# vainglorygame/analyzer

Hardware: AMD Instinct MI355X
Metric: matches/sec rated (whole node), 3v3 TrueSkill, 1M-player roster (higher is better)
Workload: dtype fp32; 1 GPU; global_batch=10000000, seq_len=6, players=1000000, matches_per_gpu=10000000, team_size=3, parallelism=dp1, mode=exact, bench_config=2, skew=1, force_merge=False

## Files before the change

### analyzer_amd/config.py

```python
from __future__ import annotations

import os
from dataclasses import dataclass, field
from typing import Mapping, Optional

BETA = 10.0 / 30 * 3000
ENV_MU = 1500.0
ENV_SIGMA = 1000.0
DRAW_PROBABILITY = 0.0

MODES = ("casual", "ranked", "blitz", "br", "5v5_casual", "5v5_ranked")
TRACK_COLUMNS = ("trueskill",) + tuple("trueskill_" + m for m in MODES)
N_TRACKS = len(TRACK_COLUMNS)
MODE_UNSUPPORTED = 255


def _env(env: Mapping[str, str], key: str) -> Optional[str]:
    v = env.get(key)
    return v if v else None


def _tristate(v: Optional[str]) -> Optional[bool]:
    if v is None or v == "" or v.lower() == "auto":
        return None
# ... 38 lines not shown
    crunch_queue: str = "crunch_global"
    dotelesuckmatch: bool = False
    telesuck_queue: str = "telesuck"
    dosewmatch: bool = False
    sew_queue: str = "sew"
    engine: str = "python"
    quarantine: bool = True
    dotelemetry: bool = False
    telemetry_events: str = "100,300"
    resident: bool = True
    synthetic_telemetry: bool = False
    telemetry_source: Optional[str] = None
    skip_rated: bool = False
    pipeline: bool = False
    fault_poison: frozenset = frozenset()
    fault_exit_after: int = 0
    cas_retries: int = 50

    @staticmethod
    def from_env(env: Mapping[str, str] = os.environ) -> "WorkerConfig":
        return WorkerConfig(
            rabbitmq_uri=_env(env, "RABBITMQ_URI") or "amqp://localhost",
            database_uri=_env(env, "DATABASE_URI"),
            batchsize=int(_env(env, "BATCHSIZE") or 500),
            chunksize=int(_env(env, "CHUNKSIZE") or 100),
            idle_timeout=float(_env(env, "IDLE_TIMEOUT") or 1),
            queue=_env(env, "QUEUE") or "analyze",
            docrunchmatch=env.get("DOCRUNCHMATCH") == "true",
            crunch_queue=_env(env, "CRUNCH_QUEUE") or "crunch_global",
            dotelesuckmatch=env.get("DOTELESUCKMATCH") == "true",
            telesuck_queue=_env(env, "TELESUCK_QUEUE") or "telesuck",
            dosewmatch=env.get("DOSEWMATCH") == "true",
            sew_queue=_env(env, "SEW_QUEUE") or "sew",
            engine=_env(env, "ENGINE") or "python",
            quarantine=(env.get("QUARANTINE") or "true") == "true",
            dotelemetry=env.get("DOTELEMETRY") == "true",
            telemetry_events=_env(env, "TELEMETRY_EVENTS") or "100,300",
            synthetic_telemetry=env.get("SYNTHETIC_TELEMETRY") == "true",
            telemetry_source=_env(env, "TELEMETRY_SOURCE"),
            resident=_resident_default(env),
            skip_rated=env.get("SKIP_RATED") == "true",
            pipeline=env.get("PIPELINE") == "true",
            fault_poison=frozenset(x for x in (env.get("FAULT_POISON") or "").split(",") if x),
            fault_exit_after=int(env.get("FAULT_EXIT_AFTER") or 0),
            cas_retries=int(env.get("CAS_RETRIES") or 50),
        )

    @property
    def failed_queue(self) -> str:
        return self.queue + "_failed"


@dataclass(frozen=True)
class EngineConfig:

    rate_blocks: int = 0
    prepass_at: float = 0.7
    prepass_at_set: bool = False
    prepass_cus: int = 0
    prepass_exclusive: bool = False
    prepass_serial: Optional[bool] = None
    roster_warm: Optional[bool] = None
    merge_bucket_mb: float = 64.0
    comm_dtype: str = ""
    sweeps: int = 1
    dist_backend: str = "nccl"
    checkpoint_every: int = 1
    checkpoint_dir: Optional[str] = None
    trace: bool = False
    check_rounds: bool = False
    rate_idle: int = 0
    rate_local: int = 1
    rate_diag: int = 0
    rate_tight: int = -1
    tele_fused_tail: int = 0
    tele_role: int = -1
    tele_fuse_max: int = 262_144

    NATIVE_KNOBS = {
        "ANA_TELE_IMPL": "telemetry aggregation: 1 one-hot MFMA GEMM (default), 0 LDS atomics",
        "ANA_SCHED_SMALL": "micro-batch schedule: hash lists (default) or bitonic sort",
        "ANA_SORT_RB / ANA_SORT_NT": "radix-sort tile rows / non-temporal loads (tuning)",
        "ANA_SCHED_RUNS": "last schedule pass: run-end table (1, default) or digit offsets + fix-up (0)",
    }

    def rate_knobs(self) -> list:
        return [self.rate_idle, self.rate_local, self.rate_diag, self.rate_tight, self.tele_fused_tail,
                self.tele_role]

    @staticmethod
    def from_env(env: Mapping[str, str] = os.environ) -> "EngineConfig":
        return EngineConfig(
            rate_blocks=int(_env(env, "ANA_RATE_BLOCKS") or 0),
            prepass_at=float(_env(env, "ANA_PREPASS_AT") or 0.7) if env.get("ANA_PREPASS_AT") != "0" else 0.0,
            prepass_at_set=bool(env.get("ANA_PREPASS_AT")),
            prepass_cus=int(_env(env, "ANA_PREPASS_CUS") or 0),
            prepass_exclusive=env.get("ANA_PREPASS_EXCLUSIVE", "0") not in ("", "0", "false"),
            prepass_serial=_tristate(env.get("ANA_PREPASS_SERIAL")),
            roster_warm=_tristate(env.get("ANA_ROSTER_WARM")),
            merge_bucket_mb=float(_env(env, "ANA_MERGE_BUCKET_MB") or 64),
            comm_dtype=_env(env, "COMM_DTYPE") or "",
            sweeps=int(_env(env, "SWEEPS") or 1),
            dist_backend=_env(env, "ANA_DIST_BACKEND") or "nccl",
            checkpoint_every=int(_env(env, "CHECKPOINT_EVERY") or 1),
            checkpoint_dir=_env(env, "CHECKPOINT_DIR"),
            trace=(env.get("ANA_TRACE") or "0") not in ("", "0"),
            check_rounds=(env.get("ANA_CHECK_ROUNDS") or "0") not in ("", "0"),
            rate_idle=int(_env(env, "ANA_RATE_IDLE") or 0),
            rate_local=int(_env(env, "ANA_RATE_LOCAL") or 1),
            rate_diag=int(_env(env, "ANA_RATE_DIAG") or 0),
            rate_tight=int(_env(env, "ANA_RATE_TIGHT") or -1),
            tele_fused_tail=int(_env(env, "ANA_TELE_FUSED_TAIL") or 0),
            tele_role=int(_env(env, "ANA_TELE_ROLE") or -1),
            tele_fuse_max=int(_env(env, "ANA_TELE_FUSE_MAX") or 262_144),
        )
```

### analyzer_amd/csrc/bindings.cpp

```cpp
#include <torch/extension.h>

#include <cstdlib>
#include <ATen/hip/HIPContext.h>

#include <algorithm>
#include <numeric>
#include <string>
#include <tuple>
#include <vector>

#include "career_core.h"
#include "common.h"
#include "gen_core.h"
#include "host.h"
#include "ingest.h"
#include "kernels.h"
#include "ladder_core.h"
#include "matchmake_core.h"
#include "select_core.h"

namespace {

using torch::Tensor;

// ... 948 lines not shown
  Tensor records = torch::empty({L, 2 * K + 2}, lobbies.options());
  if (L == 0) return {out, records};
  if (dev.is_cuda()) {
    check_hip(ana::launch_balance((int)K, lobbies.data_ptr<int32_t>(), L, state.data_ptr<float>(), at,
                                  vst.data_ptr<float>(), P, (int)mode, (float)beta2, (float)unknown_sigma,
                                  out.data_ptr<int32_t>(), records.data_ptr<int32_t>(), stream_of(lobbies)),
              "balance");
  } else {
    TORCH_CHECK(ana::host_balance((int)K, lobbies.data_ptr<int32_t>(), L, state.data_ptr<float>(), at,
                                  vst.data_ptr<float>(), P, (int)mode, (float)beta2, (float)unknown_sigma,
                                  out.data_ptr<int32_t>(), records.data_ptr<int32_t>()) == 0,
                "balance: bad arguments");
  }
  return {out, records};
}

std::vector<Tensor> queue_order(Tensor queue, Tensor state, c10::optional<Tensor> attrs, Tensor vst, int64_t mode,
                                double unknown_sigma) {
  const auto dev = queue.device();
  check(queue, "queue", torch::kInt32, dev);
  TORCH_CHECK(queue.dim() == 1 && queue.size(0) <= 0x7fffffffLL, "queue_order: queue must be [Q], Q < 2^31");
  TORCH_CHECK(mode >= 0 && mode < ana::kModes, "queue_order: mode must be 0..5");
  const float* at = matchmake_roster(state, attrs, vst, dev, "queue_order");
  const int64_t Q = queue.size(0), P = state.size(0);
  Tensor keys = torch::empty({Q}, queue.options()), vals = torch::empty({Q}, queue.options());
  if (Q == 0) return {keys, vals};
  if (!dev.is_cuda()) {
    TORCH_CHECK(ana::host_queue_keys(queue.data_ptr<int32_t>(), Q, state.data_ptr<float>(), at,
                                     vst.data_ptr<float>(), P, (int)mode, (float)unknown_sigma, u32p(keys),
                                     u32p(vals)) == 0, "queue_order: bad arguments");
    Tensor sk = torch::empty({Q}, queue.options()), sv = torch::empty({Q}, queue.options());
    const uint32_t* k = u32p(keys);
    uint32_t* order = u32p(sv);
    std::iota(order, order + Q, 0u);
    std::stable_sort(order, order + Q, [&](uint32_t a, uint32_t b) { return k[a] < k[b]; });
    for (int64_t i = 0; i < Q; ++i) u32p(sk)[i] = k[order[i]];
    return {sk, sv};
  }
  const hipStream_t s = stream_of(queue);
  check_hip(ana::launch_queue_keys(queue.data_ptr<int32_t>(), Q, state.data_ptr<float>(), at, vst.data_ptr<float>(),
                                   P, (int)mode, (float)unknown_sigma, u32p(keys), u32p(vals), s),
            "queue_keys");
  return sort_pairs_on_stream(keys, vals, Q, 32, s);
}

std::tuple<int64_t, int64_t, int64_t> matchmake_geometry(int64_t K) {
  TORCH_CHECK(K >= 1 && K <= ana::kMaxTeamSize, "matchmake_geometry: K must be 1..5");
  const int G = ana::split_group_lanes((int)K);
  return {G, 64 / G, ana::kMatchmakeThreads / G};
}

std::vector<int64_t> split_masks(int64_t K) {
  TORCH_CHECK(K >= 1 && K <= ana::kMaxTeamSize, "split_masks: K must be 1..5");
  std::vector<int64_t> out;
  ana::with_team_size((int)K, [&](auto k) {
    for (uint16_t m : ana::kSplits<decltype(k)::value>.mask) out.push_back(m);
  });
  return out;
}

void reset_tags(Tensor state) {
  const auto dev = state.device();
  const int64_t P = check_state(state, dev, "reset_tags");
  if (dev.is_cuda()) check_hip(ana::launch_reset_tags(state.data_ptr<float>(), P, stream_of(state)), "reset_tags");
  else ana::host_reset_tags(state.data_ptr<float>(), P);
}

}

void register_batch_host(pybind11::module& m);
void register_telemetry_file(pybind11::module& m);

PYBIND11_MODULE(TORCH_EXTENSION_NAME, m) {
  register_batch_host(m);
  register_telemetry_file(m);
  m.doc() = "analyzer_amd native engine: gfx950 HIP kernels + C++ host mirror";
  m.def("gen_roster", &gen_roster, "K7: synthetic roster (state [P,16], attrs [P,4])");
  m.def("gen_stream", &gen_stream, "K7: synthetic match stream rec [M, 2K+2]");
  m.def("schedule_workspace_bytes", &schedule_workspace_bytes);
  m.def("levels_device", &levels_device);
  m.def("sort_pairs", &sort_pairs, "stable LSD radix sort of int32 (key, value) pairs (device)");
  m.def("levels", &levels, "K5 host levelizer: per-match conflict-free round (0 = stateless)");
  m.def("schedule", &schedule, "K5: per-slot occurrence index (chronological order per player)");
  m.def("rate", &rate, "K1-K4/K6: exact dataflow rating of a stream");
  m.def("gen_event_counts", &gen_event_counts, "K8/K7: synthetic telemetry events per match");
  m.def("gen_events", &gen_events, "K8/K7: synthetic telemetry events (CSR by match)");
  m.def("telemetry", &telemetry, "K8: per-participant telemetry aggregation [M, 2K, 8]");
  m.attr("STAT_FEATURES") = ana::kStatFeatures;
  m.def("sweep_delta", &sweep_delta, "K9: per-rank natural-parameter messages for the DP merge");
  m.def("sweep_apply", &sweep_apply, "K9: decode summed messages against the common start (-> s, s2)",
        py::arg("s0"), py::arg("buf"), py::arg("attrs"), py::arg("s"), py::arg("s2"), py::arg("vst"),
        py::arg("unknown_sigma"), py::arg("scaled"), py::arg("clamps") = py::none());
  m.def("sweep_delta_packed", &sweep_delta_packed, "K9: messages straight into bf16/fp16 + int32 all-reduce operands");
  m.def("sweep_apply_packed", &sweep_apply_packed,
        "K9: decode bf16/fp16 + int32 summed messages (-> s, s2); with a prefix also the record-correction delta table",
        py::arg("s0"), py::arg("msg"), py::arg("cnt"), py::arg("attrs"), py::arg("s"), py::arg("s2"), py::arg("vst"),
        py::arg("unknown_sigma"), py::arg("clamps") = py::none(), py::arg("prefix") = py::none(),
        py::arg("delta") = py::none());
  m.def("correct_records", &correct_records,
        "K9: causal correction of a window's records: += the delta table of the earlier ranks' messages");
  m.def("sweep_block_reduce", &sweep_block_reduce, "K9: owner block sum (+ exclusive prefixes) of the split collective",
        py::arg("recv"), py::arg("N"), py::arg("bf16"), py::arg("total"), py::arg("pref") = py::none());
  m.def("prefix_delta", &prefix_delta, "K9: the record correction's delta table of a scaled message prefix");
  m.def("pack_rows", &pack_rows, "C2: changed rows of a round slice -> fixed-capacity [cap, 33] entries");
  m.def("check_round", &check_round, "C2 race detector: one round's matches share no player (flag |= 1)");
  m.def("unpack_rows", &unpack_rows, "C2: write gathered entries (id >= 0) into the roster, tags zeroed");
  m.def("write_record_file", &write_record_file, "P3: write a match-record file (ANAREC01)");
  py::class_<ana::RecordReader>(m, "RecordReader")
      .def(py::init<const std::string&, int64_t, int, bool>(), py::arg("path"), py::arg("window"),
           py::arg("slots") = 3, py::arg("pinned") = true)
      .def_property_readonly("K", &ana::RecordReader::K)
      .def_property_readonly("num_matches", &ana::RecordReader::num_matches)
      .def_property_readonly("window", &ana::RecordReader::window)
      .def_property_readonly("num_windows", &ana::RecordReader::num_windows)
      .def_property_readonly("pinned", &ana::RecordReader::pinned)
      .def("acquire", &reader_acquire,
           "next filled window as (slot, base, tensor view of pinned memory) or None at EOF")
      .def("release", &ana::RecordReader::release, "return the oldest acquired slot");
  m.def("cu_masked_stream", &cu_masked_stream, "HIP stream limited to N CUs (spread over XCDs), or to the others",
        py::arg("device"), py::arg("num_cus"), py::arg("invert") = false);
  m.def("progress_signal", &progress_signal, "8-B signal-memory word for the executor's tail signal");
  m.def("stream_wait_value64", &stream_wait_value64, "hipStreamWaitValue64(stream, ptr, >= value)");
  m.def("stream_write_value64", &stream_write_value64, "hipStreamWriteValue64(stream, ptr, value)");
  m.def("can_wait_value", &can_wait_value, "hipDeviceAttributeCanUseStreamWaitValue");
  m.def("reset_tags", &reset_tags, "zero the dataflow tags of a roster");
  m.def("records_digest", &records_digest, "deterministic fp64 digest of a window's packed output rows "
        "(+ its status counts added to hist)", py::arg("rows"), py::arg("K"), py::arg("scratch"),
        py::arg("out"), py::arg("hist") = py::none());
  m.def("records_digest_scratch", &records_digest_scratch, "scratch doubles of records_digest");
  m.def("records_select", &records_select, "K10: hits [n, 12] int32 of the bitmap's players in a window's records "
        "joined with its packed output rows, ascending (match, slot)", py::arg("rec"), py::arg("rows"),
        py::arg("base"), py::arg("P"), py::arg("bitmap"));
  m.def("ladder", &ladder, "K11: [order, score, rank] per track of the mask (bit t = granule t) of a roster's state: "
        "descending score, ties by ascending id, rank -1 = unranked", py::arg("state"), py::arg("mask"),
        py::arg("score"), py::arg("max_sigma"));
  m.def("preview", &preview, "K12: packed [M, 4] int32 rows (status, quality, p_win0 bits, 0) of a stream's records "
        "against the stored roster: what rate would write, read-only", py::arg("rec"), py::arg("K"), py::arg("state"),
        py::arg("attrs"), py::arg("vst"), py::arg("beta2"), py::arg("unknown_sigma"));
  m.def("balance", &balance, "K12: [packed [L, 8] int32 rows (status, split, team0, quality, p_win0, quality_given), "
        "records [L, 2K+2]] of the best split of each lobby", py::arg("lobbies"), py::arg("K"), py::arg("state"),
        py::arg("attrs"), py::arg("vst"), py::arg("mode"), py::arg("beta2"), py::arg("unknown_sigma"));
  m.def("queue_order", &queue_order, "K12: [sorted keys, queue positions] of a queue by descending mode-track prior mu "
        "(stable; failed players last with key -1)", py::arg("queue"), py::arg("state"), py::arg("attrs"),
        py::arg("vst"), py::arg("mode"), py::arg("unknown_sigma"));
  m.def("matchmake_geometry", &matchmake_geometry, "K12: (lanes per lobby, lobbies per wave, lobbies per workgroup)");
  m.def("split_masks", &split_masks, "K12: the team-0 masks of the splits of a 2K lobby, in index order");
  m.def("careers_add", &careers_add, "K13: fold one window (rec [M, 2K+2] joined with its packed rows [M, W]) into the "
        "career table [P, 16] int32 in place: careers_add(table, rec, rows, base, P, track, score, modes)");
  m.attr("CAREER_WORDS") = ana::kCareerWords;
  m.attr("CAREER_TILE") = ana::kCareerTile;
  m.attr("MAX_SLOTS") = (int64_t)ana::kMaxSlots;
  m.attr("LADDER_CONSERVATIVE") = (int)ana::kLadderConservative;
  m.attr("LADDER_MU") = (int)ana::kLadderMu;
  m.attr("HIT_WORDS") = ana::kHitWords;
  m.attr("SELECT_TILE") = ana::kSelectTile;
  m.def("emulate_allreduce", &emulate_allreduce,
        "DP pricing on one GPU: an all-reduce stand-in (buffer unchanged) on N CUs for >= us microseconds");
  m.def("warm_rows", &warm_rows, "read every roster row once (cache warm-up before a rating launch)");
  m.def("epoch_bump", &epoch_bump, "device launch epoch += 1 (graph replays)");
  m.attr("ROW_FLOATS") = ana::kRowFloats;
  m.attr("N_TRACKS") = ana::kTracks;
  m.attr("VST_TIERS") = ana::kVstTiers;
}
```

### analyzer_amd/csrc/kernels.h

```cpp
#pragma once

#include <stddef.h>
#include <stdint.h>

#include <hip/hip_runtime_api.h>

#include "common.h"
#include "gen_core.h"
#include "telemetry_core.h"

namespace ana {

int launch_gen_roster(const GenRosterParams& g, float* state, float* attrs, hipStream_t s);
int launch_gen_stream(int K, const GenStreamParams& g, int32_t* rec, int64_t M, hipStream_t s);

int launch_reset_tags(float* state, int64_t P, hipStream_t s);
int launch_warm_rows(const float* state, int64_t P, uint32_t* sink, hipStream_t s);
int launch_epoch_bump(int32_t* e, hipStream_t s);
int launch_emulate_allreduce(void* buf, int64_t bytes, int channels, int passes, double us, hipStream_t s);

size_t schedule_workspace_bytes(int64_t nslots, int64_t num_players);

size_t records_digest_scratch_doubles(int K);
int launch_records_digest(int K, const float* rows, int64_t M, int64_t W, double* scratch, double* out,
                          int64_t* hist, hipStream_t s);

constexpr int kSelectTile = 2048;
int64_t records_select_tiles(int64_t M);
int launch_records_select_count(int K, const int32_t* rec, const float* rows, int64_t W, int64_t M, int64_t P,
                                const uint32_t* bitmap, uint32_t* counts, int64_t* offsets, hipStream_t s);
int launch_records_select_emit(int K, const int32_t* rec, const float* rows, int64_t W, int64_t M, int64_t base,
                               int64_t P, const uint32_t* bitmap, const int64_t* offsets, int32_t* hits,
                               int64_t nhits, hipStream_t s);

constexpr int kLadderTile = 1024;
int launch_ladder_keys(const float* state, int64_t P, uint32_t mask, int score, float max_sigma, uint32_t* keys,
                       uint32_t* ids, int64_t stride, uint32_t* counts, hipStream_t s);
int launch_ladder_ranks(const uint32_t* keys, const uint32_t* ids, int64_t P, int64_t R, int32_t* order, float* score,
                        int32_t* rank, hipStream_t s);

int launch_preview(int K, const int32_t* rec, int64_t M, const float* state, const float* attrs, const float* vst,
                   int64_t P, float beta2, float unknown_sigma, int32_t* out, hipStream_t s);
int launch_balance(int K, const int32_t* lobbies, int64_t L, const float* state, const float* attrs,
                   const float* vst, int64_t P, int mode, float beta2, float unknown_sigma, int32_t* out,
                   int32_t* records, hipStream_t s);
int launch_queue_keys(const int32_t* queue, int64_t Q, const float* state, const float* attrs, const float* vst,
                      int64_t P, int mode, float unknown_sigma, uint32_t* keys, uint32_t* vals, hipStream_t s);

constexpr int kCareerTile = 4096;
size_t career_edge_bytes(int64_t n);
int launch_career_keys(int K, const int32_t* rec, const float* rows, int64_t W, int64_t M, int64_t P, int track,
                       int score, uint32_t modes, uint32_t* keys, uint32_t* vals, uint32_t* events, hipStream_t s);
int launch_career_fold(const uint32_t* keys, const uint32_t* vals, const uint32_t* events, int64_t n, int K,
                       int64_t base, int64_t P, int32_t* table, void* edges, hipStream_t s);

size_t radix_sort_workspace_bytes(int64_t n);
int launch_radix_sort_pairs(uint32_t* keys, uint32_t* vals, uint32_t* keys_alt, uint32_t* vals_alt,
                            int64_t n, int bits, void* ws, int* result_in_alt, hipStream_t s);
int launch_sched_sort(int K, const int32_t* rec, int64_t M, uint32_t num_players, uint32_t* ka,
                      uint32_t* va, uint32_t* kb, uint32_t* vb, void* ws, uint32_t* link,
                      hipStream_t s, int32_t* deps = nullptr, uint32_t* ctrl = nullptr, int nz = 0,
                      int32_t* epoch_bump = nullptr, int sort_nt = -1);
int launch_levels(int K, const int32_t* rec, const uint32_t* link, int32_t* deps, int32_t* pushed,
                  int32_t* level, int64_t M, int64_t P, uint32_t* ctrl, hipStream_t s);
int launch_schedule(int K, const int32_t* rec, int64_t M, int64_t P, uint32_t* link,
                    int32_t* deps, void* ws, size_t ws_bytes, uint32_t* overflow, hipStream_t s,
                    bool zero_ctrl = false, int32_t* epoch_bump = nullptr, int sort_nt = -1);

int launch_rate(int K, const int32_t* rec, const uint32_t* link, int32_t* deps, float* state,
                const float* attrs, float* first_prior, const RateOut& out, uint32_t* ctrl,
                const RateParams& prm, const TelemetryParams& tp, int blocks, hipStream_t s);


int launch_gen_event_counts(const GenEventParams& g, int64_t base, int64_t M, int64_t* counts,
                            hipStream_t s);
int launch_gen_events(int K, const GenEventParams& g, int64_t base, const int32_t* rec,
                      const int64_t* evoff, int64_t M, int32_t* events, hipStream_t s);
int tele_impl();
int launch_telemetry(int K, const TelemetryParams& tp, uint32_t* bad, hipStream_t s);

}

namespace ana {
int launch_sweep_delta(const float* s0, const float* a, const float* s, const float* attrs,
                       const float* vst, float unknown_sigma, int scaled, float* buf, int64_t P,
                       hipStream_t st);
int launch_sweep_apply(const float* s0, const float* buf, const float* attrs, float* s, float* s2,
                       const float* vst, float unknown_sigma, int scaled, int64_t P, uint32_t* clamps,
                       hipStream_t st);
int launch_sweep_delta_packed(const float* s0, const float* a, const float* s, const float* attrs,
                              const float* vst, float unknown_sigma, int bf16, void* msg, int32_t* cnt,
                              int64_t P, hipStream_t st, int64_t mstride = 7, int64_t cstride = 1);
int launch_sweep_block_reduce(const int32_t* recv, int N, int64_t blk, int bf16, int32_t* total, int32_t* pref,
                              hipStream_t st);
int launch_sweep_apply_packed(const float* s0, const void* msg, const int32_t* cnt, int bf16,
                              const float* attrs, float* s, float* s2, const float* vst, float unknown_sigma,
                              int64_t P, uint32_t* clamps, const void* prefix, float* delta, hipStream_t st,
                              int64_t mstride = 7, int64_t cstride = 1);
int launch_prefix_delta(const float* s0, const void* prefix, int bf16, const float* attrs, const float* vst,
                        float unknown_sigma, float* delta, int64_t P, hipStream_t st);
int launch_correct_records(int K, const int32_t* rec, int64_t M, float* rows, int64_t orow, const float* delta,
                           int64_t P, hipStream_t st);
int launch_pack_rows(const int32_t* rec, int K, int64_t m, const uint8_t* status, int64_t sstride,
                     const float* state, float* out, int64_t cap, hipStream_t st);
int launch_unpack_rows(const float* buf, int64_t n, float* state, hipStream_t st);
int launch_check_round(const int32_t* rec, int K, const int64_t* idx, int64_t m, int64_t P, uint32_t round,
                       unsigned long long* owner, uint32_t* flag, hipStream_t st);
}
```

### analyzer_amd/csrc/radix_sort.hip

```cpp
#include <hip/hip_runtime.h>

#include <cstdlib>

#include "common.h"
#include "kernels.h"

namespace ana {

namespace {

#ifndef ANA_SORT_THREADS
#define ANA_SORT_THREADS 512
#endif
constexpr int kThreads = ANA_SORT_THREADS;
constexpr int kWaves = kThreads / 64;
constexpr int kItems = 16;
constexpr int kTile = kThreads * kItems;
constexpr int kRadix = 256;
constexpr int kRadixMax = 1024;

__device__ __forceinline__ int64_t xcd_tile(int64_t tiles) {
  const int64_t i = blockIdx.x, q = tiles >> 3, r = tiles & 7, x = i & 7;
  return x * q + (x < r ? x : r) + (i >> 3);
}

template <int NT>
__device__ __forceinline__ uint32_t ld32(const uint32_t* p) {
  if constexpr (NT >= 1) return __builtin_nontemporal_load(p);
  else return *p;
}
template <int NT>
__device__ __forceinline__ void st32(uint32_t* p, uint32_t v) {
  if constexpr (NT == 1) __builtin_nontemporal_store(v, p);
  else *p = v;
}

__device__ __forceinline__ uint32_t block_exclusive_scan(uint32_t x, uint32_t* wsum,
                                                         uint32_t* total) {
  const int lane = threadIdx.x & 63, wv = threadIdx.x >> 6;
  uint32_t inc = x;
#pragma unroll
  for (int off = 1; off < 64; off <<= 1) {
    const uint32_t y = __shfl_up(inc, off);
    if (lane >= off) inc += y;
  }
  if (lane == 63) wsum[wv] = inc;
  __syncthreads();
  uint32_t before = 0, all = 0;
#pragma unroll
  for (int w = 0; w < kWaves; ++w) {
    if (w < wv) before += wsum[w];
    all += wsum[w];
  }
  if (total) *total = all;
  __syncthreads();
  return before + inc - x;
}

template <int KS>
__device__ __forceinline__ void decode_tile_keys(const int32_t* __restrict__ rec, uint32_t kend,
                                                 int64_t base, int64_t n, uint32_t* lk) {
  constexpr int S = 2 * KS, R = S + 2;
  const uint32_t lo = (uint32_t)base;
  const uint32_t hi = (uint32_t)(base + kTile < n ? base + kTile : n);
  const uint32_t m_lo = lo / S, m_hi = (hi + S - 1) / S;
  for (uint32_t m = m_lo + threadIdx.x; m < m_hi; m += kThreads) {
    const int32_t* src = rec + (int64_t)m * R;
    int32_t r[R];
    if constexpr (R % 4 == 0) {
#pragma unroll
      for (int k = 0; k < R / 4; ++k) {
        const int4 v = reinterpret_cast<const int4*>(src)[k];
        r[4 * k] = v.x; r[4 * k + 1] = v.y; r[4 * k + 2] = v.z; r[4 * k + 3] = v.w;
      }
    } else {
#pragma unroll
      for (int k = 0; k < R; ++k) r[k] = src[k];
    }
    const bool rates = early_status<KS>(r, (int64_t)kend) == kRated;
    const uint32_t m0 = (uint32_t)r[S];
#pragma unroll
    for (int j = 0; j < S; ++j) {
      const uint32_t slot = m * S + j;
      const int pos = j < KS ? j : j - KS;
      const bool in_roster = pos < (j < KS ? meta_n0(m0) : meta_n1(m0));
      if (slot >= lo && slot < hi) lk[slot - lo] = rates && in_roster ? (uint32_t)r[j] : kend;
    }
  }
}

struct SchedInit {
  int32_t* deps = nullptr;
  uint32_t* ctrl = nullptr;
  int nz = 0;
  int32_t* epoch_bump = nullptr;
};

template <int KS, int RB = 8, int NT = 0>
__global__ void __launch_bounds__(kThreads)
radix_upsweep(const uint32_t* __restrict__ keys, const int32_t* __restrict__ rec, uint32_t kend,
              int64_t n, int shift, uint32_t* __restrict__ counts, int64_t tiles, SchedInit init = {}) {
  constexpr int kR = 1 << RB;
  __shared__ uint32_t hist[kWaves][kR];
  __shared__ uint32_t lkeys[KS > 0 ? kTile : 1];
  const int tid = threadIdx.x, wv = tid >> 6;
  for (int i = tid; i < kWaves * kR; i += kThreads) (&hist[0][0])[i] = 0u;
  const int64_t tile = xcd_tile(tiles);
  const int64_t base = tile * kTile;
  if constexpr (KS > 0) {
    if (init.deps) {
      constexpr int S = 2 * KS;
      const int64_t hi = base + kTile < n ? base + kTile : n;
      for (int64_t m = (base + S - 1) / S + tid; m < (hi + S - 1) / S; m += kThreads) init.deps[m] = 0;
    }
    if (blockIdx.x == 0) {
      if (tid < init.nz) init.ctrl[tid] = 0u;
      if (tid == 0 && init.epoch_bump) init.epoch_bump[0] += 1;
    }
  }
  if constexpr (KS > 0) decode_tile_keys<KS>(rec, kend, base, n, lkeys);
  __syncthreads();
#pragma unroll
  for (int k = 0; k < kItems; ++k) {
    const int64_t idx = base + k * kThreads + tid;
    if (idx < n) {
      const uint32_t key = KS > 0 ? lkeys[k * kThreads + tid] : ld32<NT>(keys + idx);
      atomicAdd(&hist[wv][(key >> shift) & (kR - 1)], 1u);
    }
  }
  __syncthreads();
#pragma unroll
  for (int d = tid; d < kR; d += kThreads) {
    uint32_t c = 0;
#pragma unroll
    for (int w = 0; w < kWaves; ++w) c += hist[w][d];
    counts[(int64_t)d * tiles + tile] = c;
  }
}

template <int DPT>
__device__ __forceinline__ void digits_exclusive_scan(uint32_t (&v)[DPT], uint32_t* wsum,
                                                      uint32_t* total) {
  uint32_t s = 0;
#pragma unroll
  for (int j = 0; j < DPT; ++j) {
    const uint32_t x = v[j];
    v[j] = s;
    s += x;
  }
  const uint32_t before = block_exclusive_scan(s, wsum, total);
#pragma unroll
  for (int j = 0; j < DPT; ++j) v[j] += before;
}

__global__ void __launch_bounds__(kThreads)
radix_rowscan(uint32_t* __restrict__ counts, int64_t tiles, uint32_t* __restrict__ totals) {
  __shared__ uint32_t wsum[kWaves];
  constexpr int kPer = 4;
  uint32_t* row = counts + (int64_t)blockIdx.x * tiles;
  uint32_t carry = 0;
  for (int64_t start = 0; start < tiles; start += kThreads * kPer) {
    uint32_t v[kPer], s = 0;
#pragma unroll
    for (int q = 0; q < kPer; ++q) {
      const int64_t t = start + (int64_t)threadIdx.x * kPer + q;
      v[q] = t < tiles ? row[t] : 0u;
      s += v[q];
    }
    uint32_t all;
    uint32_t ex = carry + block_exclusive_scan(s, wsum, &all);
#pragma unroll
    for (int q = 0; q < kPer; ++q) {
      const int64_t t = start + (int64_t)threadIdx.x * kPer + q;
      if (t < tiles) row[t] = ex;
      ex += v[q];
    }
    carry += all;
  }
  if (threadIdx.x == 0) totals[blockIdx.x] = carry;
}

struct RunEnds {
  uint32_t kf, vf, kl, vl;
};
constexpr uint32_t kRunEmpty = 0xffffffffu;

template <int KS, bool LINK, int RB = 8, int NT = 0>
__global__ void __launch_bounds__(kThreads)
radix_downsweep(const uint32_t* __restrict__ kin, const uint32_t* __restrict__ vin,
                const int32_t* __restrict__ rec, uint32_t kend,
                uint32_t* __restrict__ kout, uint32_t* __restrict__ vout, int64_t n, int shift,
                const uint32_t* __restrict__ counts, const uint32_t* __restrict__ totals,
                int64_t tiles, int slots_per_match, uint32_t* __restrict__ link,
                uint32_t vlo = 0u, uint32_t vhi = 0xffffffffu, int bounds = 1,
                RunEnds* __restrict__ bnd = nullptr, int nd = 0) {
  constexpr int kR = 1 << RB;
  constexpr int DPT = kR >= kThreads ? kR / kThreads : 1;
  static_assert(kR % kThreads == 0 || kThreads % kR == 0, "radix and block must divide");
  __shared__ uint32_t skey[kTile];
  __shared__ uint32_t sval[kTile];
  __shared__ uint32_t wcnt[kWaves][kR];
  __shared__ uint32_t tstart[kR];
  __shared__ uint32_t gstart[kR];
  __shared__ uint32_t wsum[kWaves];
  const int tid = threadIdx.x, lane = tid & 63, wv = tid >> 6;
  const int64_t tile = xcd_tile(tiles);
  const int64_t base = tile * kTile;
  for (int i = tid; i < kWaves * kR; i += kThreads) (&wcnt[0][0])[i] = 0u;
  const bool local_ends = LINK && bnd != nullptr;
  if (!local_ends) {
    uint32_t v[DPT];
#pragma unroll
    for (int j = 0; j < DPT; ++j) v[j] = tid * DPT + j < kR ? totals[tid * DPT + j] : 0u;
    digits_exclusive_scan<DPT>(v, wsum, nullptr);
#pragma unroll
    for (int j = 0; j < DPT; ++j)
      if (tid * DPT + j < kR) gstart[tid * DPT + j] = v[j] + counts[(int64_t)(tid * DPT + j) * tiles + tile];
  }
  if constexpr (KS > 0) decode_tile_keys<KS>(rec, kend, base, n, sval);
  __syncthreads();

  const uint64_t lt_mask = (1ull << lane) - 1ull;
  uint32_t key[kItems], val[kItems], rank[kItems];
#pragma unroll
  for (int it = 0; it < kItems; ++it) {
    const int64_t idx = base + (int64_t)(wv * kItems + it) * 64 + lane;
    const bool valid = idx < n;
    if constexpr (KS > 0) key[it] = valid ? sval[(wv * kItems + it) * 64 + lane] : 0xffffffffu;
    else key[it] = valid ? ld32<NT>(kin + idx) : 0xffffffffu;
    if constexpr (KS == 0) val[it] = valid ? ld32<NT>(vin + idx) : 0u;
    else val[it] = (uint32_t)idx;
  }
#pragma unroll
  for (int it = 0; it < kItems; ++it) {
    const uint32_t d = (key[it] >> shift) & (kR - 1);
    uint64_t peers = ~0ull;
#pragma unroll
    for (int b = 0; b < RB; ++b) {
      const uint64_t bal = __ballot((d >> b) & 1u);
      peers &= ((d >> b) & 1u) ? bal : ~bal;
    }
    const uint32_t before = (uint32_t)__popcll(peers & lt_mask);
    const uint32_t run = wcnt[wv][d];
    rank[it] = run + before;
    if (before == (uint32_t)__popcll(peers) - 1u) wcnt[wv][d] = run + (uint32_t)__popcll(peers);
  }
  __syncthreads();
  {
    uint32_t v[DPT];
#pragma unroll
    for (int j = 0; j < DPT; ++j) {
      const int d = tid * DPT + j;
      uint32_t s = 0;
      if (d < kR) {
#pragma unroll
        for (int w = 0; w < kWaves; ++w) {
          const uint32_t c = wcnt[w][d];
          wcnt[w][d] = s;
          s += c;
        }
      }
      v[j] = s;
    }
    digits_exclusive_scan<DPT>(v, wsum, nullptr);
#pragma unroll
    for (int j = 0; j < DPT; ++j)
      if (tid * DPT + j < kR) tstart[tid * DPT + j] = v[j];
  }
  __syncthreads();
#pragma unroll
  for (int it = 0; it < kItems; ++it) {
    const uint32_t d = (key[it] >> shift) & (kR - 1);
    const uint32_t pos = tstart[d] + wcnt[wv][d] + rank[it];
    skey[pos] = key[it];
    sval[pos] = val[it];
  }
  __syncthreads();
  const int64_t nvalid = n - base < kTile ? n - base : kTile;
  if constexpr (LINK) {
    if (local_ends && bounds && tid < nd) {
      const uint32_t e = tid + 1 < kR ? tstart[tid + 1] : (uint32_t)kTile;
      if (tstart[tid] == e) bnd[tile * nd + tid].kf = kRunEmpty;
    }
  }
#pragma unroll
  for (int k = 0; k < kItems; ++k) {
    const int i = k * kThreads + tid;
    if (i < nvalid) {
      const uint32_t kk = skey[i];
      const uint32_t d = (kk >> shift) & (kR - 1);
      const int64_t o = local_ends ? 0 : (int64_t)gstart[d] + (i - (int64_t)tstart[d]);
      if constexpr (!LINK) {
        st32<NT>(kout + o, kk);
        st32<NT>(vout + o, sval[i]);
      } else {
        const int hi = d + 1 < (uint32_t)kR ? (int)tstart[d + 1] : kTile;
        const bool first = i == (int)tstart[d];
        const bool last = i + 1 == hi || i + 1 >= nvalid;
        const uint32_t v = sval[i];
        if (bounds && (first || last)) {
          if (local_ends) {
            if ((int)d < nd) {
              RunEnds* r = bnd + tile * nd + d;
              if (first) { r->kf = kk; r->vf = v; }
              if (last) { r->kl = kk; r->vl = v; }
            }
          } else {
            st32<NT>(kout + o, kk);
            st32<NT>(vout + o, v);
          }
        }
        if (kk < kend && v >= vlo && v < vhi) {
          uint32_t w = (!last && skey[i + 1] == kk) ? sval[i + 1] / (uint32_t)slots_per_match
                                                     : kNoMatch;
          if (!first && skey[i - 1] == kk) w |= kLinkHasPred;
          st32<NT>(link + v, w);
        }
      }
    }
  }
}

static bool local_runs() {
  const char* e = getenv("ANA_SCHED_RUNS");
  return !(e && atoi(e) == 0);
}

static int link_parts(int64_t n) {
  if (const char* e = getenv("ANA_LINK_PARTS")) {
    const int v = atoi(e);
    if (v >= 1) return v > 16 ? 16 : v;
  }
  const int64_t bytes = n * 4, part = 256ll << 20;
  return (int)((bytes + part - 1) / part);
}

template <int RB = 8>
__global__ void __launch_bounds__(kThreads)
sched_fixup(const uint32_t* __restrict__ kout, const uint32_t* __restrict__ vout, int64_t n,
            uint32_t kend, const uint32_t* __restrict__ counts, const uint32_t* __restrict__ totals,
            int64_t tiles, int slots_per_match, uint32_t* __restrict__ link) {
  constexpr int kR = 1 << RB;
  __shared__ uint32_t wsum[kWaves];
  const int d = blockIdx.y;
  const uint32_t tot = totals[d];
  if (tot == 0) return;
  uint32_t below = 0;
#pragma unroll
  for (int j = threadIdx.x; j < kR; j += kThreads) below += j < d ? totals[j] : 0u;
  uint32_t all = 0;
  const uint32_t before = block_exclusive_scan(below, wsum, &all);
  (void)before;
  const uint32_t dstart = all;
  const int64_t t = (int64_t)blockIdx.x * kThreads + threadIdx.x;
  if (t >= tiles) return;
  const uint32_t* row = counts + (int64_t)d * tiles;
  const uint32_t c0 = row[t];
  const uint32_t c1 = t + 1 < tiles ? row[t + 1] : tot;
  if (c1 == c0) return;
  const int64_t of = (int64_t)dstart + c0, ol = (int64_t)dstart + c1 - 1;
  const uint32_t kf = kout[of], kl = kout[ol];
  const bool pred = kf < kend && of > 0 && kout[of - 1] == kf;
  const bool succ = kl < kend && ol + 1 < n && kout[ol + 1] == kl;
  const uint32_t nxt = succ ? vout[ol + 1] / (uint32_t)slots_per_match : kNoMatch;
  if (of == ol) {
    if (kf < kend) link[vout[of]] = nxt | (pred ? kLinkHasPred : 0u);
    return;
  }
  if (pred) {
    const uint32_t v = vout[of];
    link[v] |= kLinkHasPred;
  }
  if (succ) {
    const uint32_t v = vout[ol];
    link[v] = (link[v] & ~kMatchMask) | nxt;
  }
}

constexpr int kRunsMaxDigits = 32;

__global__ void __launch_bounds__(kThreads)
sched_runs_last(const RunEnds* __restrict__ bnd, int64_t tiles, int nd, int32_t* __restrict__ seglast) {
  __shared__ int32_t wmax[kWaves];
  const int d = blockIdx.y;
  const int64_t t = (int64_t)blockIdx.x * kThreads + threadIdx.x;
  int32_t x = (t < tiles && bnd[t * nd + d].kf != kRunEmpty) ? (int32_t)t : -1;
#pragma unroll
  for (int off = 32; off >= 1; off >>= 1) x = max(x, __shfl_xor(x, off));
  if ((threadIdx.x & 63) == 0) wmax[threadIdx.x >> 6] = x;
  __syncthreads();
  if (threadIdx.x == 0) {
    int32_t m = wmax[0];
#pragma unroll
    for (int w = 1; w < kWaves; ++w) m = max(m, wmax[w]);
    seglast[(int64_t)d * gridDim.x + blockIdx.x] = m;
  }
}

__global__ void __launch_bounds__(kThreads)
sched_runs_fixup(const RunEnds* __restrict__ bnd, int64_t tiles, int nd, const int32_t* __restrict__ seglast,
                 uint32_t kend, int slots_per_match, uint32_t* __restrict__ link) {
  __shared__ int32_t wmax[kWaves];
  __shared__ int32_t carry_s;
  const int d = blockIdx.y, lane = threadIdx.x & 63, wv = threadIdx.x >> 6;
  const int64_t seg = blockIdx.x;
  if (wv == 0) {
    int32_t c = -1;
    for (int64_t q = lane; q < seg; q += 64) c = max(c, seglast[(int64_t)d * gridDim.x + q]);
#pragma unroll
    for (int off = 32; off >= 1; off >>= 1) c = max(c, __shfl_xor(c, off));
    if (lane == 0) carry_s = c;
  }
  const int64_t t = seg * kThreads + threadIdx.x;
  RunEnds me = {kRunEmpty, 0u, kRunEmpty, 0u};
  if (t < tiles) me = bnd[t * nd + d];
  const bool full = me.kf != kRunEmpty;
  int32_t x = full ? (int32_t)t : -1;
#pragma unroll
  for (int off = 1; off < 64; off <<= 1) {
    const int32_t y = __shfl_up(x, off);
    if (lane >= off) x = max(x, y);
  }
  if (lane == 63) wmax[wv] = x;
  __syncthreads();
  int32_t before = carry_s;
  for (int w = 0; w < wv; ++w) before = max(before, wmax[w]);
  int32_t ex = __shfl_up(x, 1);
  ex = lane == 0 ? -1 : ex;
  const int32_t pred = max(before, ex);
  if (!full || pred < 0 || me.kf >= kend) return;
  const RunEnds pr = bnd[(int64_t)pred * nd + d];
  if (pr.kl != me.kf) return;
  atomicOr(&link[me.vf], kLinkHasPred);
  atomicAnd(&link[pr.vl], ~kMatchMask | (me.vf / (uint32_t)slots_per_match));
}

}

size_t radix_sort_workspace_bytes(int64_t n) {
  const int64_t tiles = (n + kTile - 1) / kTile;
  return (size_t)(tiles * kRadixMax + kRadixMax) * 4;
}

int launch_radix_sort_pairs(uint32_t* keys, uint32_t* vals, uint32_t* keys_alt, uint32_t* vals_alt,
                            int64_t n, int bits, void* ws, int* result_in_alt, hipStream_t s) {
  *result_in_alt = 0;
  if (n <= 0) return 0;
  if (n > 0x7fffffffLL || bits < 1 || bits > 32) return (int)hipErrorInvalidValue;
  const int64_t tiles = (n + kTile - 1) / kTile;
  uint32_t* counts = static_cast<uint32_t*>(ws);
  uint32_t* totals = counts + tiles * kRadix;
  uint32_t *ki = keys, *vi = vals, *ko = keys_alt, *vo = vals_alt;
  for (int shift = 0; shift < bits; shift += 8) {
    hipLaunchKernelGGL(radix_upsweep<0>, dim3((unsigned)tiles), dim3(kThreads), 0, s, ki, nullptr,
                       0u, n, shift, counts, tiles);
    hipLaunchKernelGGL(radix_rowscan, dim3(kRadix), dim3(kThreads), 0, s, counts, tiles, totals);
    hipLaunchKernelGGL((radix_downsweep<0, false>), dim3((unsigned)tiles), dim3(kThreads), 0, s, ki,
                       vi, nullptr, 0u, ko, vo, n, shift, counts, totals, tiles, 1, nullptr);
    std::swap(ki, ko);
    std::swap(vi, vo);
    *result_in_alt ^= 1;
  }
  return (int)hipGetLastError();
}

template <int K, int RB, int NT>
static void sched_sort_k(const int32_t* rec, int64_t n, uint32_t kend, int bits, uint32_t* ka,
                         uint32_t* va, uint32_t* kb, uint32_t* vb, uint32_t* counts,
                         int64_t tiles, uint32_t* link, const SchedInit& init, hipStream_t s) {
  constexpr int S = 2 * K;
  constexpr int kR = 1 << RB;
  uint32_t* totals = counts + tiles * kR;
  const dim3 grid((unsigned)tiles), block(kThreads);
  const uint32_t *ki = nullptr, *vi = nullptr;
  uint32_t *ko = kb, *vo = vb;
  for (int shift = 0; shift < bits; shift += RB) {
    const bool first = shift == 0, last = shift + RB >= bits;
    const int nd = bits - shift < RB ? 1 << (bits - shift) : kR;
    if (last && !first && nd <= kRunsMaxDigits && local_runs()) {
      RunEnds* bnd = reinterpret_cast<RunEnds*>(counts);
      const int64_t nseg = (tiles + kThreads - 1) / kThreads;
      int32_t* seglast = reinterpret_cast<int32_t*>(bnd + tiles * nd);
      const int parts = link_parts(n);
      for (int q = 0; q < parts; ++q)
        hipLaunchKernelGGL((radix_downsweep<0, true, RB, NT>), grid, block, 0, s, ki, vi, nullptr, kend, ko, vo,
                           n, shift, counts, totals, tiles, S, link, (uint32_t)(n * q / parts),
                           (uint32_t)(n * (q + 1) / parts), q == 0 ? 1 : 0, bnd, nd);
      const dim3 sgrid((unsigned)nseg, (unsigned)nd);
      hipLaunchKernelGGL(sched_runs_last, sgrid, block, 0, s, bnd, tiles, nd, seglast);
      hipLaunchKernelGGL(sched_runs_fixup, sgrid, block, 0, s, bnd, tiles, nd, seglast, kend, S, link);
      break;
    }
    if (first)
      hipLaunchKernelGGL((radix_upsweep<K, RB, NT>), grid, block, 0, s, nullptr, rec, kend, n, shift, counts, tiles,
                         init);
    else
      hipLaunchKernelGGL((radix_upsweep<0, RB, NT>), grid, block, 0, s, ki, nullptr, kend, n, shift, counts, tiles);
    hipLaunchKernelGGL(radix_rowscan, dim3(kR), block, 0, s, counts, tiles, totals);
    const int parts = last ? link_parts(n) : 1;
    if (first && last)
      for (int q = 0; q < parts; ++q)
        hipLaunchKernelGGL((radix_downsweep<K, true, RB, NT>), grid, block, 0, s, nullptr, nullptr, rec, kend, ko,
                           vo, n, shift, counts, totals, tiles, S, link, (uint32_t)(n * q / parts),
                           (uint32_t)(n * (q + 1) / parts), q == 0 ? 1 : 0);
    else if (first)
      hipLaunchKernelGGL((radix_downsweep<K, false, RB, NT>), grid, block, 0, s, nullptr, nullptr, rec, kend, ko,
                         vo, n, shift, counts, totals, tiles, S, nullptr);
    else if (last)
      for (int q = 0; q < parts; ++q)
        hipLaunchKernelGGL((radix_downsweep<0, true, RB, NT>), grid, block, 0, s, ki, vi, nullptr, kend, ko, vo,
                           n, shift, counts, totals, tiles, S, link, (uint32_t)(n * q / parts),
                           (uint32_t)(n * (q + 1) / parts), q == 0 ? 1 : 0);
    else
      hipLaunchKernelGGL((radix_downsweep<0, false, RB, NT>), grid, block, 0, s, ki, vi, nullptr, kend, ko, vo, n,
                         shift, counts, totals, tiles, S, nullptr);
    if (last)
      hipLaunchKernelGGL((sched_fixup<RB>), dim3((unsigned)((tiles + kThreads - 1) / kThreads), kR), block,
                         0, s, ko, vo, n, kend, counts, totals, tiles, S, link);
    ki = ko;
    vi = vo;
    ko = ko == kb ? ka : kb;
    vo = vo == vb ? va : vb;
  }
}

int launch_sched_sort(int K, const int32_t* rec, int64_t M, uint32_t num_players, uint32_t* ka,
                      uint32_t* va, uint32_t* kb, uint32_t* vb, void* ws, uint32_t* link,
                      hipStream_t s, int32_t* deps, uint32_t* ctrl, int nz, int32_t* epoch_bump,
                      int sort_nt) {
  const int64_t n = M * 2 * K;
  if (n <= 0) return 0;
  if (n > kMaxSlots) return (int)hipErrorInvalidValue;
  int bits = 1;
  while (bits < 32 && (1ull << bits) <= (uint64_t)num_players) ++bits;
  const int64_t tiles = (n + kTile - 1) / kTile;
  uint32_t* counts = static_cast<uint32_t*>(ws);
  SchedInit init;
  init.deps = deps;
  init.ctrl = ctrl;
  init.nz = ctrl ? nz : 0;
  init.epoch_bump = epoch_bump;
  const char* rb_e = getenv("ANA_SORT_RB");
  const char* nt_e = getenv("ANA_SORT_NT");
  const int rb_env = rb_e ? atoi(rb_e) : 8;
  const int nt = nt_e ? atoi(nt_e) : sort_nt >= 0 ? sort_nt : 0;
  const bool wide = bits <= 20 && rb_env == 10;
  const bool known = with_team_size(K, [&](auto k) {
    constexpr int kK = decltype(k)::value;
    if (wide) sched_sort_k<kK, 10, 0>(rec, n, num_players, bits, ka, va, kb, vb, counts, tiles, link, init, s);
    else if (nt == 1) sched_sort_k<kK, 8, 1>(rec, n, num_players, bits, ka, va, kb, vb, counts, tiles, link, init, s);
    else if (nt == 2) sched_sort_k<kK, 8, 2>(rec, n, num_players, bits, ka, va, kb, vb, counts, tiles, link, init, s);
    else sched_sort_k<kK, 8, 0>(rec, n, num_players, bits, ka, va, kb, vb, counts, tiles, link, init, s);
  });
  return known ? (int)hipGetLastError() : (int)hipErrorInvalidValue;
}

}
```

Before: 1.592 billion matches/s.

## Pack schedule radix-sort pairs into 5 bytes with position-implied sorted digits

Adds a packed path to the three-pass schedule radix sort. Intermediate keys are stored as a single byte, with the already-sorted digit recovered from each element's position against per-digit start offsets, and the top key bits are folded into the upper bits of the value word. Each pass then moves 5 bytes per pair instead of 8, which cuts memory traffic in a bandwidth-bound sort. The cost is extra digit-lookup work (ballot/popcount and a while loop) in the downsweep. The path also needs the key bits minus 16 plus the slot bits to fit in 32 bits; it is on by default and can be disabled with ANA_SORT_PACK=0.

```diff
diff --git a/analyzer_amd/config.py b/analyzer_amd/config.py
--- a/analyzer_amd/config.py
+++ b/analyzer_amd/config.py
@@ -144,6 +144,8 @@
         "ANA_SCHED_SMALL": "micro-batch schedule: hash lists (default) or bitonic sort",
         "ANA_SORT_RB / ANA_SORT_NT": "radix-sort tile rows / non-temporal loads (tuning)",
         "ANA_SCHED_RUNS": "last schedule pass: run-end table (1, default) or digit offsets + fix-up (0)",
+        "ANA_SORT_PACK": "three-pass schedule sort: 5-byte pairs, sorted digit implied by position "
+                         "(1, default) or two-word pairs (0)",
     }
 
     def rate_knobs(self) -> list:
diff --git a/analyzer_amd/csrc/bindings.cpp b/analyzer_amd/csrc/bindings.cpp
--- a/analyzer_amd/csrc/bindings.cpp
+++ b/analyzer_amd/csrc/bindings.cpp
@@ -1054,6 +1054,12 @@
   m.def("sort_pairs", &sort_pairs, "stable LSD radix sort of int32 (key, value) pairs (device)");
   m.def("levels", &levels, "K5 host levelizer: per-match conflict-free round (0 = stateless)");
   m.def("schedule", &schedule, "K5: per-slot occurrence index (chronological order per player)");
+  m.def("sched_sort_packed",
+        [](int64_t nslots, int64_t num_players) {
+          TORCH_CHECK(num_players >= 1 && num_players < 0x7fffffffLL, "num_players out of range");
+          return ana::sched_sort_packed(nslots, (uint32_t)num_players);
+        },
+        "K5: whether the device schedule of nslots slots sorts 5-byte pairs (radix_sort.hip)");
   m.def("rate", &rate, "K1-K4/K6: exact dataflow rating of a stream");
   m.def("gen_event_counts", &gen_event_counts, "K8/K7: synthetic telemetry events per match");
   m.def("gen_events", &gen_events, "K8/K7: synthetic telemetry events (CSR by match)");
diff --git a/analyzer_amd/csrc/kernels.h b/analyzer_amd/csrc/kernels.h
--- a/analyzer_amd/csrc/kernels.h
+++ b/analyzer_amd/csrc/kernels.h
@@ -61,6 +61,7 @@
                       uint32_t* va, uint32_t* kb, uint32_t* vb, void* ws, uint32_t* link,
                       hipStream_t s, int32_t* deps = nullptr, uint32_t* ctrl = nullptr, int nz = 0,
                       int32_t* epoch_bump = nullptr, int sort_nt = -1);
+bool sched_sort_packed(int64_t nslots, uint32_t num_players);
 int launch_levels(int K, const int32_t* rec, const uint32_t* link, int32_t* deps, int32_t* pushed,
                   int32_t* level, int64_t M, int64_t P, uint32_t* ctrl, hipStream_t s);
 int launch_schedule(int K, const int32_t* rec, int64_t M, int64_t P, uint32_t* link,
diff --git a/analyzer_amd/csrc/radix_sort.hip b/analyzer_amd/csrc/radix_sort.hip
--- a/analyzer_amd/csrc/radix_sort.hip
+++ b/analyzer_amd/csrc/radix_sort.hip
@@ -33,6 +33,21 @@
 __device__ __forceinline__ void st32(uint32_t* p, uint32_t v) {
   if constexpr (NT == 1) __builtin_nontemporal_store(v, p);
   else *p = v;
+}
+
+typedef uint32_t u32x4 __attribute__((ext_vector_type(4)));
+template <int NT>
+__device__ __forceinline__ u32x4 ld128(const uint8_t* p) {
+  const u32x4* q = reinterpret_cast<const u32x4*>(p);
+  if constexpr (NT >= 1) return __builtin_nontemporal_load(q);
+  else return *q;
+}
+
+__device__ __forceinline__ uint32_t digit_at(const uint32_t* ps, uint32_t g, int lane) {
+  uint32_t c = 0;
+#pragma unroll
+  for (int j = 0; j < 256 / 64; ++j) c += (uint32_t)__popcll(__ballot(ps[j * 64 + lane] <= g));
+  return c - 1u;
 }
 
 __device__ __forceinline__ uint32_t block_exclusive_scan(uint32_t x, uint32_t* wsum,
@@ -96,7 +111,7 @@
   int32_t* epoch_bump = nullptr;
 };
 
-template <int KS, int RB = 8, int NT = 0>
+template <int KS, int RB = 8, int NT = 0, bool BYTES = false>
 __global__ void __launch_bounds__(kThreads)
 radix_upsweep(const uint32_t* __restrict__ keys, const int32_t* __restrict__ rec, uint32_t kend,
               int64_t n, int shift, uint32_t* __restrict__ counts, int64_t tiles, SchedInit init = {}) {
@@ -120,12 +135,23 @@
   }
   if constexpr (KS > 0) decode_tile_keys<KS>(rec, kend, base, n, lkeys);
   __syncthreads();
-#pragma unroll
-  for (int k = 0; k < kItems; ++k) {
-    const int64_t idx = base + k * kThreads + tid;
-    if (idx < n) {
-      const uint32_t key = KS > 0 ? lkeys[k * kThreads + tid] : ld32<NT>(keys + idx);
-      atomicAdd(&hist[wv][(key >> shift) & (kR - 1)], 1u);
+  if constexpr (BYTES) {
+    static_assert(kItems == 16 && KS == 0 && RB == 8, "one 16-B load per thread");
+    const int64_t off = base + (int64_t)tid * kItems;
+    if (off < n) {
+      const u32x4 q = ld128<NT>(reinterpret_cast<const uint8_t*>(keys) + off);
+#pragma unroll
+      for (int b = 0; b < kItems; ++b)
+        if (off + b < n) atomicAdd(&hist[wv][(q[b >> 2] >> (8 * (b & 3))) & 255u], 1u);
+    }
+  } else {
+#pragma unroll
+    for (int k = 0; k < kItems; ++k) {
+      const int64_t idx = base + k * kThreads + tid;
+      if (idx < n) {
+        const uint32_t key = KS > 0 ? lkeys[k * kThreads + tid] : ld32<NT>(keys + idx);
+        atomicAdd(&hist[wv][(key >> shift) & (kR - 1)], 1u);
+      }
     }
   }
   __syncthreads();
@@ -185,7 +211,7 @@
 };
 constexpr uint32_t kRunEmpty = 0xffffffffu;
 
-template <int KS, bool LINK, int RB = 8, int NT = 0>
+template <int KS, bool LINK, int RB = 8, int NT = 0, int PACK = 0>
 __global__ void __launch_bounds__(kThreads)
 radix_downsweep(const uint32_t* __restrict__ kin, const uint32_t* __restrict__ vin,
                 const int32_t* __restrict__ rec, uint32_t kend,
@@ -193,21 +219,38 @@
                 const uint32_t* __restrict__ counts, const uint32_t* __restrict__ totals,
                 int64_t tiles, int slots_per_match, uint32_t* __restrict__ link,
                 uint32_t vlo = 0u, uint32_t vhi = 0xffffffffu, int bounds = 1,
-                RunEnds* __restrict__ bnd = nullptr, int nd = 0) {
+                RunEnds* __restrict__ bnd = nullptr, int nd = 0,
+                const uint32_t* __restrict__ pstart = nullptr, uint32_t* __restrict__ keep_start = nullptr,
+                int slot_bits = 0) {
   constexpr int kR = 1 << RB;
   constexpr int DPT = kR >= kThreads ? kR / kThreads : 1;
   static_assert(kR % kThreads == 0 || kThreads % kR == 0, "radix and block must divide");
-  __shared__ uint32_t skey[kTile];
+  static_assert(PACK == 0 || (RB == 8 && kItems == 16), "packed pairs: 8-bit digits, 16-B byte loads");
+  static_assert(PACK == 0 || (PACK == 1 && KS > 0 && !LINK) || (PACK == 2 && KS == 0 && !LINK) ||
+                (PACK == 3 && KS == 0 && LINK), "packed pairs: pass 0, pass 1, link pass");
+  __shared__ __align__(16) uint32_t skey[kTile];
   __shared__ uint32_t sval[kTile];
   __shared__ uint32_t wcnt[kWaves][kR];
   __shared__ uint32_t tstart[kR];
   __shared__ uint32_t gstart[kR];
+  __shared__ uint32_t pdig[PACK >= 2 ? kR : 1];
   __shared__ uint32_t wsum[kWaves];
   const int tid = threadIdx.x, lane = tid & 63, wv = tid >> 6;
   const int64_t tile = xcd_tile(tiles);
   const int64_t base = tile * kTile;
   for (int i = tid; i < kWaves * kR; i += kThreads) (&wcnt[0][0])[i] = 0u;
   const bool local_ends = LINK && bnd != nullptr;
+  uint32_t key[kItems], val[kItems], rank[kItems];
+  u32x4 stage = {0u, 0u, 0u, 0u};
+  if constexpr (PACK >= 2) {
+    const int64_t off = base + (int64_t)tid * kItems;
+    if (off < n) stage = ld128<NT>(reinterpret_cast<const uint8_t*>(kin) + off);
+#pragma unroll
+    for (int it = 0; it < kItems; ++it) {
+      const int64_t idx = base + (int64_t)(wv * kItems + it) * 64 + lane;
+      val[it] = idx < n ? ld32<NT>(vin + idx) : 0u;
+    }
+  }
   if (!local_ends) {
     uint32_t v[DPT];
 #pragma unroll
@@ -215,21 +258,51 @@
     digits_exclusive_scan<DPT>(v, wsum, nullptr);
 #pragma unroll
     for (int j = 0; j < DPT; ++j)
-      if (tid * DPT + j < kR) gstart[tid * DPT + j] = v[j] + counts[(int64_t)(tid * DPT + j) * tiles + tile];
+      if (tid * DPT + j < kR) {
+        if (PACK != 0 && keep_start && blockIdx.x == 0) keep_start[tid * DPT + j] = v[j];
+        gstart[tid * DPT + j] = v[j] + counts[(int64_t)(tid * DPT + j) * tiles + tile];
+      }
   }
   if constexpr (KS > 0) decode_tile_keys<KS>(rec, kend, base, n, sval);
-  __syncthreads();
-
+  if constexpr (PACK >= 2) {
+    for (int i = tid; i < kR; i += kThreads) pdig[i] = pstart[i];
+    reinterpret_cast<u32x4*>(skey)[tid] = stage;
+  }
   const uint64_t lt_mask = (1ull << lane) - 1ull;
-  uint32_t key[kItems], val[kItems], rank[kItems];
-#pragma unroll
-  for (int it = 0; it < kItems; ++it) {
-    const int64_t idx = base + (int64_t)(wv * kItems + it) * 64 + lane;
-    const bool valid = idx < n;
-    if constexpr (KS > 0) key[it] = valid ? sval[(wv * kItems + it) * 64 + lane] : 0xffffffffu;
-    else key[it] = valid ? ld32<NT>(kin + idx) : 0xffffffffu;
-    if constexpr (KS == 0) val[it] = valid ? ld32<NT>(vin + idx) : 0u;
-    else val[it] = (uint32_t)idx;
+  __syncthreads();
+
+  if constexpr (PACK >= 2) {
+    const uint32_t p0 = (uint32_t)(base + (int64_t)wv * kItems * 64);
+    const uint32_t d0 = digit_at(pdig, p0, lane), d1 = digit_at(pdig, p0 + kItems * 64 - 1, lane);
+    uint32_t dcur = d0;
+#pragma unroll
+    for (int it = 0; it < kItems; ++it) {
+      const uint32_t g = p0 + it * 64 + lane;
+      const bool valid = g < n;
+      uint32_t dl = dcur;
+      if (d0 != d1) {
+        while (dl + 1u < (uint32_t)kR && pdig[dl + 1u] <= g) ++dl;
+        dcur = __shfl(dl, 63);
+      }
+      const uint32_t b = reinterpret_cast<const uint8_t*>(skey)[(wv * kItems + it) * 64 + lane];
+      const uint32_t w = val[it];
+      if constexpr (PACK == 2) {
+        key[it] = valid ? (dl | b << 8) : 0xffffffffu;
+      } else {
+        key[it] = valid ? (b | dl << 8 | (w >> slot_bits) << 16) : 0xffffffffu;
+        val[it] = w & ((1u << slot_bits) - 1u);
+      }
+    }
+  } else {
+#pragma unroll
+    for (int it = 0; it < kItems; ++it) {
+      const int64_t idx = base + (int64_t)(wv * kItems + it) * 64 + lane;
+      const bool valid = idx < n;
+      if constexpr (KS > 0) key[it] = valid ? sval[(wv * kItems + it) * 64 + lane] : 0xffffffffu;
+      else key[it] = valid ? ld32<NT>(kin + idx) : 0xffffffffu;
+      if constexpr (KS == 0) val[it] = valid ? ld32<NT>(vin + idx) : 0u;
+      else val[it] = (uint32_t)idx;
+    }
   }
 #pragma unroll
   for (int it = 0; it < kItems; ++it) {
@@ -290,7 +363,13 @@
       const uint32_t kk = skey[i];
       const uint32_t d = (kk >> shift) & (kR - 1);
       const int64_t o = local_ends ? 0 : (int64_t)gstart[d] + (i - (int64_t)tstart[d]);
-      if constexpr (!LINK) {
+      if constexpr (!LINK && PACK == 1) {
+        reinterpret_cast<uint8_t*>(kout)[o] = (uint8_t)(kk >> 8);
+        st32<NT>(vout + o, sval[i] | (kk >> 16) << slot_bits);
+      } else if constexpr (!LINK && PACK == 2) {
+        reinterpret_cast<uint8_t*>(kout)[o] = (uint8_t)kk;
+        st32<NT>(vout + o, sval[i]);
+      } else if constexpr (!LINK) {
         st32<NT>(kout + o, kk);
         st32<NT>(vout + o, sval[i]);
       } else {
@@ -326,6 +405,23 @@
   return !(e && atoi(e) == 0);
 }
 
+static bool pack_pairs() {
+  const char* e = getenv("ANA_SORT_PACK");
+  return !(e && atoi(e) == 0);
+}
+
+static int ceil_log2(int64_t n) {
+  int b = 0;
+  while ((1ll << b) < n) ++b;
+  return b;
+}
+
+static int key_bits(uint32_t num_players) {
+  int bits = 1;
+  while (bits < 32 && (1ull << bits) <= (uint64_t)num_players) ++bits;
+  return bits;
+}
+
 static int link_parts(int64_t n) {
   if (const char* e = getenv("ANA_LINK_PARTS")) {
     const int v = atoi(e);
@@ -467,13 +563,42 @@
 template <int K, int RB, int NT>
 static void sched_sort_k(const int32_t* rec, int64_t n, uint32_t kend, int bits, uint32_t* ka,
                          uint32_t* va, uint32_t* kb, uint32_t* vb, uint32_t* counts,
-                         int64_t tiles, uint32_t* link, const SchedInit& init, hipStream_t s) {
+                         int64_t tiles, uint32_t* link, const SchedInit& init, hipStream_t s,
+                         bool pack = false) {
   constexpr int S = 2 * K;
   constexpr int kR = 1 << RB;
   uint32_t* totals = counts + tiles * kR;
   const dim3 grid((unsigned)tiles), block(kThreads);
   const uint32_t *ki = nullptr, *vi = nullptr;
   uint32_t *ko = kb, *vo = vb;
+  if constexpr (RB == 8) {
+    if (pack) {
+      const int slot_bits = ceil_log2(n), nd = 1 << (bits - 16);
+      uint32_t *start0 = totals + kR, *start1 = totals + 2 * kR;
+      hipLaunchKernelGGL((radix_upsweep<K, 8, NT>), grid, block, 0, s, nullptr, rec, kend, n, 0, counts, tiles, init);
+      hipLaunchKernelGGL(radix_rowscan, dim3(kR), block, 0, s, counts, tiles, totals);
+      hipLaunchKernelGGL((radix_downsweep<K, false, 8, NT, 1>), grid, block, 0, s, nullptr, nullptr, rec, kend, kb,
+                         vb, n, 0, counts, totals, tiles, S, nullptr, 0u, 0xffffffffu, 1, nullptr, 0, nullptr,
+                         start0, slot_bits);
+      hipLaunchKernelGGL((radix_upsweep<0, 8, NT, true>), grid, block, 0, s, kb, nullptr, kend, n, 8, counts, tiles);
+      hipLaunchKernelGGL(radix_rowscan, dim3(kR), block, 0, s, counts, tiles, totals);
+      hipLaunchKernelGGL((radix_downsweep<0, false, 8, NT, 2>), grid, block, 0, s, kb, vb, nullptr, kend, ka, va, n,
+                         8, counts, totals, tiles, S, nullptr, 0u, 0xffffffffu, 1, nullptr, 0, start0, start1,
+                         slot_bits);
+      RunEnds* bnd = reinterpret_cast<RunEnds*>(counts);
+      const int64_t nseg = (tiles + kThreads - 1) / kThreads;
+      int32_t* seglast = reinterpret_cast<int32_t*>(bnd + tiles * nd);
+      const int parts = link_parts(n);
+      for (int q = 0; q < parts; ++q)
+        hipLaunchKernelGGL((radix_downsweep<0, true, 8, NT, 3>), grid, block, 0, s, ka, va, nullptr, kend, kb, vb,
+                           n, 16, counts, totals, tiles, S, link, (uint32_t)(n * q / parts),
+                           (uint32_t)(n * (q + 1) / parts), q == 0 ? 1 : 0, bnd, nd, start1, nullptr, slot_bits);
+      const dim3 sgrid((unsigned)nseg, (unsigned)nd);
+      hipLaunchKernelGGL(sched_runs_last, sgrid, block, 0, s, bnd, tiles, nd, seglast);
+      hipLaunchKernelGGL(sched_runs_fixup, sgrid, block, 0, s, bnd, tiles, nd, seglast, kend, S, link);
+      return;
+    }
+  }
   for (int shift = 0; shift < bits; shift += RB) {
     const bool first = shift == 0, last = shift + RB >= bits;
     const int nd = bits - shift < RB ? 1 << (bits - shift) : kR;
@@ -531,8 +656,7 @@
   const int64_t n = M * 2 * K;
   if (n <= 0) return 0;
   if (n > kMaxSlots) return (int)hipErrorInvalidValue;
-  int bits = 1;
-  while (bits < 32 && (1ull << bits) <= (uint64_t)num_players) ++bits;
+  const int bits = key_bits(num_players);
   const int64_t tiles = (n + kTile - 1) / kTile;
   uint32_t* counts = static_cast<uint32_t*>(ws);
   SchedInit init;
@@ -545,14 +669,24 @@
   const int rb_env = rb_e ? atoi(rb_e) : 8;
   const int nt = nt_e ? atoi(nt_e) : sort_nt >= 0 ? sort_nt : 0;
   const bool wide = bits <= 20 && rb_env == 10;
+  const bool pack = sched_sort_packed(n, num_players);
   const bool known = with_team_size(K, [&](auto k) {
     constexpr int kK = decltype(k)::value;
     if (wide) sched_sort_k<kK, 10, 0>(rec, n, num_players, bits, ka, va, kb, vb, counts, tiles, link, init, s);
-    else if (nt == 1) sched_sort_k<kK, 8, 1>(rec, n, num_players, bits, ka, va, kb, vb, counts, tiles, link, init, s);
-    else if (nt == 2) sched_sort_k<kK, 8, 2>(rec, n, num_players, bits, ka, va, kb, vb, counts, tiles, link, init, s);
-    else sched_sort_k<kK, 8, 0>(rec, n, num_players, bits, ka, va, kb, vb, counts, tiles, link, init, s);
+    else if (nt == 1) sched_sort_k<kK, 8, 1>(rec, n, num_players, bits, ka, va, kb, vb, counts, tiles, link, init, s, pack);
+    else if (nt == 2) sched_sort_k<kK, 8, 2>(rec, n, num_players, bits, ka, va, kb, vb, counts, tiles, link, init, s, pack);
+    else sched_sort_k<kK, 8, 0>(rec, n, num_players, bits, ka, va, kb, vb, counts, tiles, link, init, s, pack);
   });
   return known ? (int)hipGetLastError() : (int)hipErrorInvalidValue;
 }
 
-}
+bool sched_sort_packed(int64_t n, uint32_t num_players) {
+  const int bits = key_bits(num_players);
+  const char* rb_e = getenv("ANA_SORT_RB");
+  if (bits <= 20 && rb_e && atoi(rb_e) == 10) return false;
+  if (bits <= 16 || (1 << (bits - 16)) > kRunsMaxDigits) return false;
+  if (!local_runs() || !pack_pairs()) return false;
+  return n >= 1 && n <= kMaxSlots && (bits - 16) + ceil_log2(n) <= 32;
+}
+
+}
```

After: 1.588 billion matches/s (median of 5 runs). About the same (-0.2%).
